# kije/gpu_raytracer

Hardware: AMD Instinct MI355X
Metric: Mrays/s (higher is better)
Workload: dtype f32

## Files before the change

### gpu_raytracer_amd/csrc/wavefront.hip

```cpp
#include "wavefront.h"
#include <cstdlib>

#include <algorithm>

#include "device_common.h"

using namespace rtdev;

#ifndef RT_WF_REFILL
#define RT_WF_REFILL 16
#endif
#ifndef RT_WF_CHUNK
#define RT_WF_CHUNK 256
#endif
#ifndef RT_WF_ADAPTIVE_CHUNK
#define RT_WF_ADAPTIVE_CHUNK 1
#endif
#ifndef RT_WF_WINDOW
#define RT_WF_WINDOW 512
#endif
#ifndef RT_WF_BLOCK_MAJOR
#define RT_WF_BLOCK_MAJOR 1
#endif
#ifndef RT_WF_SHADE_WAVES
// ... 346 lines not shown
        unsigned long long n0 = wave_sum(cnt.nodes), n1 = wave_sum(cnt.tris);
        for (int off = 32; off > 0; off >>= 1) sp_max = max(sp_max, __shfl_down(sp_max, off, WAVE));
        if (lane == 0) {
            atomicAdd(&wb.totals[rt::WF_TOTAL_NODE_VISITS], n0);
            atomicAdd(&wb.totals[rt::WF_TOTAL_TRI_TESTS], n1);
            atomicMax(&wb.totals[rt::WF_TOTAL_STACK_MAX], (unsigned long long)sp_max);
            atomicAdd(&wb.totals[rt::WF_TOTAL_NODE_STEPS], (unsigned long long)d_node_steps);
            atomicAdd(&wb.totals[rt::WF_TOTAL_LEAF_STEPS], (unsigned long long)d_leaf_steps);
            atomicAdd(&wb.totals[rt::WF_TOTAL_LEAF_LANES], (unsigned long long)d_leaf_lanes);
            atomicAdd(&wb.totals[rt::WF_TOTAL_LEAF_TRIPS], (unsigned long long)d_leaf_trips);
            atomicAdd(&wb.totals[rt::WF_TOTAL_REFILLS], (unsigned long long)d_refills);
        }
        const unsigned long long e0 = wave_sum(d_empty), e1 = wave_sum(d_entered);
        if (lane == 0) {
            atomicAdd(&wb.totals[rt::WF_TOTAL_EMPTY_VISITS], e0);
            atomicAdd(&wb.totals[rt::WF_TOTAL_CHILDREN_ENTERED], e1);
        }
    }
}

#ifndef RT_BEAM_STACK
#define RT_BEAM_STACK 512
#endif
#ifndef RT_BEAM_LEAVES
#define RT_BEAM_LEAVES 1024
#endif
#ifndef RT_BEAM_MARGIN_PX
#define RT_BEAM_MARGIN_PX 0.125f
#endif
#ifndef RT_BEAM_SAMPLES_PER_WAVE
#define RT_BEAM_SAMPLES_PER_WAVE 8u
#endif
#ifndef RT_BEAM_DIST_SCALE
#define RT_BEAM_DIST_SCALE 0.99999f
#endif
#ifndef RT_BEAM_EARLY_OUT
#define RT_BEAM_EARLY_OUT 1
#endif
#ifndef RT_BEAM_TRI_CULL
#define RT_BEAM_TRI_CULL 1
#endif
struct BeamPlanes {
    V3 n[4];
    V3 o;
};
__device__ __forceinline__ bool beam_outside(const BeamPlanes& bp, const float lo[3], const float hi[3]) {
    bool outside = false;
    for (int k = 0; k < 4; k++) {
        const V3 pv = v3((bp.n[k].x > 0.0f ? hi[0] : lo[0]) - bp.o.x, (bp.n[k].y > 0.0f ? hi[1] : lo[1]) - bp.o.y, (bp.n[k].z > 0.0f ? hi[2] : lo[2]) - bp.o.z);
        outside = outside || dot(bp.n[k], pv) < 0.0f;
    }
    return outside;
}
__device__ __forceinline__ float beam_box_distance(const V3 o, const float lo[3], const float hi[3]) {
    const float dx = fmaxf(fmaxf(lo[0] - o.x, o.x - hi[0]), 0.0f), dy = fmaxf(fmaxf(lo[1] - o.y, o.y - hi[1]), 0.0f), dz = fmaxf(fmaxf(lo[2] - o.z, o.z - hi[2]), 0.0f);
    return sqrtf(dx * dx + dy * dy + dz * dz) * RT_BEAM_DIST_SCALE;
}
__global__ __launch_bounds__(WAVE) void k_wf_beams(DevScene sc, DevFrame fr, rt::WfBuffers wb) {
    __shared__ uint32_t s_nodes[RT_BEAM_STACK];
    __shared__ uint32_t s_leaf[RT_BEAM_LEAVES];
    __shared__ uint32_t s_ref[RT_BEAM_CAP];
    __shared__ float s_dist[RT_BEAM_CAP];
    const uint32_t lane = threadIdx.x, b = blockIdx.x;
    const PixelCoord p0 = block_pixel_at(fr, b, 0);
    const float x0 = (float)p0.x - RT_BEAM_MARGIN_PX, x1 = (float)p0.x + 8.0f + RT_BEAM_MARGIN_PX;
    const float y0 = (float)p0.y - RT_BEAM_MARGIN_PX, y1 = (float)p0.y + 8.0f + RT_BEAM_MARGIN_PX;
    const DevCamera& cam = fr.cam;
    auto dir = [&](float sx, float sy) {
        const float u = sx / cam.width_f, v = sy / cam.height_f;
        const float cx = (u * 2.0f - 1.0f) * cam.aspect * cam.fov_scale, cy = (1.0f - v * 2.0f) * cam.fov_scale;
        return ld3(cam.forward) + ld3(cam.right) * cx + ld3(cam.true_up) * cy;
    };
    const V3 cs[4] = {dir(x0, y0), dir(x1, y0), dir(x1, y1), dir(x0, y1)};
    const V3 cc = dir(0.5f * (x0 + x1), 0.5f * (y0 + y1));
    BeamPlanes bp;
    bp.o = ld3(cam.origin);
    bool bad = false;
    for (int k = 0; k < 4; k++) {
        bp.n[k] = cross(cs[k], cs[(k + 1) & 3]);
        const float s = dot(bp.n[k], cc);
        if (s < 0.0f) bp.n[k] = -bp.n[k];
        for (int j = 0; j < 4; j++)
            bad = bad || !(dot(bp.n[k], cs[j]) >= -1e-6f * (fabsf(bp.n[k].x) + fabsf(bp.n[k].y) + fabsf(bp.n[k].z)) * (fabsf(cs[j].x) + fabsf(cs[j].y) + fabsf(cs[j].z)));
        bad = bad || !(fabsf(s) > 0.0f) || !(fabsf(s) < RT_F32_MAX);
    }
    uint32_t n_stack = 0, n_leaf = 0;
    bool overflow = bad;
    if (sc.n_nodes) {
        if (lane == 0) s_nodes[0] = 0u;
        n_stack = 1;
    }
    __syncthreads();
    const uint32_t slot = lane & 7u;
    const unsigned long long lower = (1ull << lane) - 1ull;
    while (n_stack > 0 && !overflow) {
        const uint32_t take = min(n_stack, 8u), base = n_stack - take;
        const bool have = (lane >> 3) < take;
        const uint32_t node = have ? s_nodes[base + (lane >> 3)] : 0u;
        __syncthreads();
        n_stack = base;
        bool inner = false, leaf = false;
        uint32_t ref = 0;
        if (have) {
            const DevNode8& nd = sc.nodes[node];
            const uint32_t ex = nd.ex_imask, imask = ex >> 24, lmask = nd.lmask & 0xFFu;
            if (((imask | lmask) >> slot) & 1u) {
                float lo[3], hi[3];
                for (int a = 0; a < 3; a++) {
                    const float sca = ldexpf(1.0f, (int)(int8_t)((ex >> (8 * a)) & 0xFFu));
                    const float ql = (float)((nd.qlo[a][slot >> 2] >> (8u * (slot & 3u))) & 0xFFu), qh = (float)((nd.qhi[a][slot >> 2] >> (8u * (slot & 3u))) & 0xFFu);
                    lo[a] = nd.org[a] + ql * sca;
                    hi[a] = nd.org[a] + qh * sca;
                    const float pad = (fabsf(lo[a]) + fabsf(hi[a])) * 2.0e-6f + 1.0e-30f;
                    lo[a] -= pad;
                    hi[a] += pad;
                }
                if (!beam_outside(bp, lo, hi)) {
                    const uint32_t below = (1u << slot) - 1u;
                    if ((imask >> slot) & 1u) {
                        inner = true;
                        ref = nd.child_base + (uint32_t)__popc(imask & below);
                    } else {
                        leaf = true;
                        ref = nd.tri_base + RT_DEV_LEAF_STRIDE * (uint32_t)__popc(lmask & below);
                    }
                }
            }
        }
        const unsigned long long mi = __ballot(inner), ml = __ballot(leaf);
        const uint32_t pi = n_stack + (uint32_t)__popcll(mi & lower), pc = n_leaf + (uint32_t)__popcll(ml & lower);
        if (inner && pi < RT_BEAM_STACK) s_nodes[pi] = ref;
        if (leaf && pc < RT_BEAM_LEAVES) s_leaf[pc] = ref;
        n_stack += (uint32_t)__popcll(mi);
        n_leaf += (uint32_t)__popcll(ml);
        overflow = n_stack > RT_BEAM_STACK || n_leaf > RT_BEAM_LEAVES;
        __syncthreads();
    }
    uint32_t n_tri = 0;
    for (uint32_t l0 = 0; l0 < n_leaf && !overflow; l0 += WAVE) {
        const uint32_t li = l0 + lane;
        uint32_t first = 0, count = 0;
        if (li < n_leaf) {
            first = s_leaf[li];
            count = sc.tris[first].leaf_count;
        }
        for (uint32_t k = 0; k < RT_DEV_LEAF_STRIDE; k++) {
            bool keep = false;
            float dist = 0.0f;
            if (k < count) {
                const DevTri& t = sc.tris[first + k];
                float lo[3], hi[3];
                for (int a = 0; a < 3; a++) {
                    const float va = t.v0[a], vb = t.v0[a] + t.e1[a], vc = t.v0[a] + t.e2[a];
                    lo[a] = fminf(va, fminf(vb, vc));
                    hi[a] = fmaxf(va, fmaxf(vb, vc));
                    const float pad = (fabsf(lo[a]) + fabsf(hi[a])) * 2.0e-6f + 1.0e-30f;
                    lo[a] -= pad;
                    hi[a] += pad;
                }
                keep = !RT_BEAM_TRI_CULL || !(lo[0] <= hi[0] && lo[1] <= hi[1] && lo[2] <= hi[2]) || !beam_outside(bp, lo, hi);
                dist = beam_box_distance(bp.o, lo, hi);
                if (!(dist >= 0.0f)) dist = 0.0f;
            }
            const unsigned long long mk = __ballot(keep);
            const uint32_t pos = n_tri + (uint32_t)__popcll(mk & lower);
            if (keep && pos < RT_BEAM_CAP) {
                s_ref[pos] = first + k;
                s_dist[pos] = dist;
            }
            n_tri += (uint32_t)__popcll(mk);
        }
        overflow = n_tri > RT_BEAM_CAP;
    }
    __syncthreads();
    if (overflow) {
        if (lane == 0) wb.beam_count[b] = RT_BEAM_OVERFLOW | atomicAdd(&wb.beam_count[wb.n_blocks], 1u);
        return;
    }
    for (uint32_t i = lane; i < n_tri; i += WAVE) {
        const float di = s_dist[i];
        uint32_t rank = 0;
        for (uint32_t j = 0; j < n_tri; j++) {
            const float dj = s_dist[j];
            rank += (dj < di || (dj == di && j < i)) ? 1u : 0u;
        }
        wb.beam_ref[(size_t)b * RT_BEAM_CAP + rank] = s_ref[i];
        wb.beam_dist[(size_t)b * RT_BEAM_CAP + rank] = di;
    }
    if (lane == 0) wb.beam_count[b] = n_tri;
}

template <bool COUNT>
__global__ __launch_bounds__(WAVE) void k_wf_trace_camera(DevScene sc, rt::WfBuffers wb, uint32_t n_samples) {
    extern __shared__ uint4 s_cam[];
    if (wb.totals[rt::WF_TOTAL_ERROR] != 0ull) return;
    const uint32_t lane = threadIdx.x;
    float* s_d = reinterpret_cast<float*>(s_cam + RT_BEAM_CAP * 3u);
    Counts cnt = {0u, 0u};
    const uint32_t chunks = (n_samples + RT_BEAM_SAMPLES_PER_WAVE - 1u) / RT_BEAM_SAMPLES_PER_WAVE;
    for (uint32_t item = blockIdx.x; item < wb.n_blocks * chunks; item += gridDim.x) {
        const uint32_t b = item / chunks, k_first = (item - b * chunks) * RT_BEAM_SAMPLES_PER_WAVE, k_end = min(n_samples, k_first + RT_BEAM_SAMPLES_PER_WAVE);
        const uint32_t n_list = (uint32_t)__builtin_amdgcn_readfirstlane((int)wb.beam_count[b]);
        if (n_list & RT_BEAM_OVERFLOW) continue;
        {
            __syncthreads();
            for (uint32_t i = lane; i < n_list; i += WAVE) {
                const uint32_t slot = wb.beam_ref[(size_t)b * RT_BEAM_CAP + i];
                const uint4* __restrict__ rec = reinterpret_cast<const uint4*>(sc.tris + slot);
                const uint4 q0 = rec[0], q1 = rec[1], q2 = rec[2];
                s_cam[3u * i] = q0;
                s_cam[3u * i + 1u] = q1;
                s_cam[3u * i + 2u] = make_uint4(q2.x, q2.y, q2.z, slot);
                s_d[i] = wb.beam_dist[(size_t)b * RT_BEAM_CAP + i];
            }
            __syncthreads();
        }
        for (uint32_t k = k_first; k < k_end; k++) {
            const uint32_t sb = RT_WF_BLOCK_MAJOR ? b * n_samples + k : k * wb.n_blocks + b;
            const uint32_t p = sb * WAVE + lane;
            const bool valid = wb.pxy[p] != 0xFFFFFFFFu;
            if (__ballot(valid) == 0ull) continue;
            V3 o = v3(0.0f, 0.0f, 0.0f), d = v3(0.0f, 0.0f, 1.0f);
            if (valid) {
                float4 ro = wb.ray_o[p], rd = wb.ray_d[p];
                RT_KEEP4_EARLY(ro);
                RT_KEEP4_EARLY(rd);
                o = f4v(ro);
                d = f4v(rd);
            }
            Hit hit;
            hit.t = valid ? RT_F32_MAX : -1.0f;
            hit.prim = RT_PRIM_MISS;
            hit.slot = 0;
            if (valid) test_spheres(sc, o, d, hit, RT_MIN_RAY_DISTANCE);
            {
                for (uint32_t i = 0; i < n_list; i++) {
                    if (RT_BEAM_EARLY_OUT && __ballot(s_d[i] < hit.t) == 0ull) break;
                    const uint4 q0 = s_cam[3u * i], q1 = s_cam[3u * i + 1u], q2 = s_cam[3u * i + 2u];
                    if (COUNT && valid) cnt.tris++;
                    float t = 0.0f;
                    const bool inside = moller_trumbore(v3(__uint_as_float(q0.x), __uint_as_float(q0.y), __uint_as_float(q0.z)), v3(__uint_as_float(q0.w), __uint_as_float(q1.x), __uint_as_float(q1.y)),
                                                        v3(__uint_as_float(q1.z), __uint_as_float(q1.w), __uint_as_float(q2.x)), o, d, t);
                    const uint32_t prim = q2.z;
                    const bool accept = inside && t > RT_MIN_RAY_DISTANCE && (t < hit.t || (t == hit.t && prim < hit.prim && hit.prim < RT_PRIM_SPHERE_FLAG));
                    hit.t = accept ? t : hit.t;
                    hit.prim = accept ? prim : hit.prim;
                    hit.slot = accept ? q2.w : hit.slot;
                }
            }
            if (COUNT && wb.probe == 2u && valid) {
                Hit h2;
                h2.t = RT_F32_MAX;
                h2.prim = RT_PRIM_MISS;
                h2.slot = 0;
                Counts c2 = {0u, 0u};
                test_spheres(sc, o, d, h2, RT_MIN_RAY_DISTANCE);
                traverse<false, false>(sc, o, d, reinterpret_cast<uint2*>(s_cam + RT_BEAM_CAP * 4u) + lane, h2, c2, RT_MIN_RAY_DISTANCE);
                if (h2.prim != hit.prim || h2.t != hit.t) {
                    if (atomicAdd(&wb.totals[rt::WF_TOTAL_EMPTY_VISITS], 1ull) == 0ull) {
                        wb.totals[rt::WF_TOTAL_NODE_STEPS] = b;
                        wb.totals[rt::WF_TOTAL_LEAF_STEPS] = ((unsigned long long)hit.prim << 32) | h2.prim;
                        wb.totals[rt::WF_TOTAL_LEAF_LANES] = ((unsigned long long)__float_as_uint(hit.t) << 32) | __float_as_uint(h2.t);
                        wb.totals[rt::WF_TOTAL_LEAF_TRIPS] = ((unsigned long long)n_list << 32) | h2.slot;
                        wb.totals[rt::WF_TOTAL_REFILLS] = p;
                    }
                }
            }
            if (valid) {
                const V3 hp = o + d * hit.t;
                const uint32_t code = hit.prim == RT_PRIM_MISS ? RT_PRIM_MISS : ((hit.prim & RT_PRIM_SPHERE_FLAG) ? hit.prim : hit.slot);
                wb.hit[p] = make_uint4(__float_as_uint(hp.x), __float_as_uint(hp.y), __float_as_uint(hp.z), code);
            }
        }
    }
    if (COUNT) {
        const unsigned long long n0 = wave_sum(cnt.nodes), n1 = wave_sum(cnt.tris);
        if (lane == 0) {
            atomicAdd(&wb.totals[rt::WF_TOTAL_NODE_VISITS], n0);
            atomicAdd(&wb.totals[rt::WF_TOTAL_TRI_TESTS], n1);
        }
    }
}

#define RT_KEEP4(v) asm volatile("" : "+v"((v).x), "+v"((v).y), "+v"((v).z), "+v"((v).w))
__device__ __forceinline__ void stage_lights(DevLight* __restrict__ s_lights, const DevScene& sc) {
    const uint32_t words = sc.n_lights * (uint32_t)(sizeof(DevLight) / 4);
    const uint32_t* __restrict__ src = reinterpret_cast<const uint32_t*>(sc.lights);
    uint32_t* dst = reinterpret_cast<uint32_t*>(s_lights);
    for (uint32_t i = threadIdx.x; i < words; i += blockDim.x) dst[i] = src[i];
    __syncthreads();
}
__device__ __forceinline__ DevMaterial load_material(const DevScene& sc, uint32_t material_id) {
    const float4* p = reinterpret_cast<const float4*>(sc.materials + material_id);
    float4 a = p[0], b = p[1];
    RT_KEEP4(a);
    RT_KEEP4(b);
    DevMaterial m;
    m.albedo[0] = a.x; m.albedo[1] = a.y; m.albedo[2] = a.z; m.metallic = a.w;
    m.emission[0] = b.x; m.emission[1] = b.y; m.emission[2] = b.z; m.ior = b.w;
    const float2 c = *reinterpret_cast<const float2*>(reinterpret_cast<const float*>(sc.materials + material_id) + 8);
    m.transmission = c.x; m.roughness = c.y;
    m._pad[0] = m._pad[1] = 0.0f;
    return m;
}

#ifndef RT_WF_GRID_WALK
#define RT_WF_GRID_WALK 31
#endif
static_assert(EXT_EPS == RT_SG_EXT_EPS, "the light grids' dilation is derived from the shadow segments' origin offset");
static_assert(RT_WF_GRID_WALK < RT_SG_SORTED_PREFIX, "a walk may only look at the ordered part of a list");
#ifndef RT_WF_GRID_BLOCKS_PER_CU
#define RT_WF_GRID_BLOCKS_PER_CU 32
#endif
#ifndef RT_WF_GRID_MIN_WAVES
#define RT_WF_GRID_MIN_WAVES 7
#endif
enum : uint32_t { GRID_VISIBLE = 0u, GRID_OCCLUDED = 1u, GRID_FORWARD = 2u, GRID_PENDING = 3u };
struct GridPending {
    V3 o, d;
    float dist, limit;
    uint32_t at;
    uint32_t i, count;
};
static_assert(RT_SG_BLOCK_ENTRIES == 2u, "grid_segment_head tests the block's two entries by name");
template <bool COUNT>
__device__ __forceinline__ uint32_t grid_segment_head(const DevScene& sc, const DevLight& light, const DevShadowGrid& g, V3 point, V3 normal, GridPending& pend,
                                                      uint32_t& n_tests, uint32_t& n_entries) {
    V3 d;
    float dist;
    shadow_segment(light, point, d, dist);
    const V3 o = point + normal * EXT_EPS;
    Hit hit;
    hit.t = dist;
    hit.prim = RT_PRIM_MISS;
    hit.slot = 0;
    test_spheres(sc, o, d, hit, RT_MIN_RAY_DISTANCE);
    if (hit.prim != RT_PRIM_MISS) return GRID_OCCLUDED;
    const uint32_t kind = g.kind;
    uint32_t cell = 0xFFFFFFFFu;
    float limit = 0.0f;
    if (kind == RT_SG_KIND_CUBE) {
        const float wx = -d.x, wy = -d.y, wz = -d.z;
        const float ax = fabsf(wx), ay = fabsf(wy), az = fabsf(wz);
        const uint32_t a = (ax >= ay && ax >= az) ? 0u : (ay >= az ? 1u : 2u);
        const float wa = a == 0u ? wx : (a == 1u ? wy : wz), wb_ = a == 0u ? wy : (a == 1u ? wz : wx), wc = a == 0u ? wz : (a == 1u ? wx : wy);
        const float inv = __builtin_amdgcn_rcpf(fabsf(wa));
        const float fu = (wb_ * inv + 1.0f) * g.scale, fv = (wc * inv + 1.0f) * g.scale;
        const uint32_t top = g.res - 1u;
        const uint32_t ix = min((uint32_t)max((int)floorf(fu), 0), top), iy = min((uint32_t)max((int)floorf(fv), 0), top);
        cell = ((2u * a + (wa < 0.0f ? 1u : 0u)) * g.res + iy) * g.res + ix;
        limit = dist + g.limit_margin;
    } else if (kind == RT_SG_KIND_ORTHO) {
        const float fu = (dot(o, ld3(g.axis_u)) - g.u0) * g.scale, fv = (dot(o, ld3(g.axis_v)) - g.v0) * g.scale;
        const float r = (float)g.res;
        if (fu >= 0.0f && fu < r && fv >= 0.0f && fv < r) cell = (uint32_t)fv * g.res + (uint32_t)fu;
        limit = (g.key_top - dot(o, ld3(g.axis_w))) + g.limit_margin;
    } else {
        return GRID_FORWARD;
    }
    if (cell == 0xFFFFFFFFu && g.near_begin == g.near_end) return GRID_VISIBLE;
    uint4 hd = make_uint4(0u, 0u, 0x7F800000u, 0u), q0 = hd, q1 = hd, q2 = hd;
    const uint4* __restrict__ blk = g.blocks + (size_t)(cell == 0xFFFFFFFFu ? 0u : cell) * RT_SG_BLOCK_QUADS;
    if (cell != 0xFFFFFFFFu) {
        hd = blk[0];
        q0 = blk[1], q1 = blk[2], q2 = blk[3];
        RT_KEEP4(hd);
        RT_KEEP4(q0);
        RT_KEEP4(q1);
        RT_KEEP4(q2);
    }
    const uint32_t count = hd.x;
    if (count > g.heavy) return GRID_FORWARD;
    const uint4* __restrict__ ovf = g.overflow;
    for (uint32_t k = g.near_begin; k < g.near_end; k++) {
        const uint4 n0 = ovf[3 * (size_t)k], n1 = ovf[3 * (size_t)k + 1], n2 = ovf[3 * (size_t)k + 2];
        if (COUNT) n_tests++;
        float t;
        if (moller_trumbore(v3(__uint_as_float(n0.y), __uint_as_float(n0.z), __uint_as_float(n0.w)), v3(__uint_as_float(n1.x), __uint_as_float(n1.y), __uint_as_float(n1.z)),
                            v3(__uint_as_float(n1.w), __uint_as_float(n2.x), __uint_as_float(n2.y)), o, d, t) &&
            t > RT_MIN_RAY_DISTANCE && t < dist)
            return GRID_OCCLUDED;
    }
    if (count == 0u || !(__uint_as_float(q0.x) < limit)) return GRID_VISIBLE;
    float t;
    if (COUNT) n_entries++, n_tests++;
    if (moller_trumbore(v3(__uint_as_float(q0.y), __uint_as_float(q0.z), __uint_as_float(q0.w)), v3(__uint_as_float(q1.x), __uint_as_float(q1.y), __uint_as_float(q1.z)),
                        v3(__uint_as_float(q1.w), __uint_as_float(q2.x), __uint_as_float(q2.y)), o, d, t) &&
        t > RT_MIN_RAY_DISTANCE && t < dist)
        return GRID_OCCLUDED;
    if (count == 1u) return GRID_VISIBLE;
    q0 = blk[4], q1 = blk[5], q2 = blk[6];
    if (!(__uint_as_float(q0.x) < limit)) return GRID_VISIBLE;
    if (COUNT) n_entries++, n_tests++;
    if (moller_trumbore(v3(__uint_as_float(q0.y), __uint_as_float(q0.z), __uint_as_float(q0.w)), v3(__uint_as_float(q1.x), __uint_as_float(q1.y), __uint_as_float(q1.z)),
                        v3(__uint_as_float(q1.w), __uint_as_float(q2.x), __uint_as_float(q2.y)), o, d, t) &&
        t > RT_MIN_RAY_DISTANCE && t < dist)
        return GRID_OCCLUDED;
    if (count == 2u || !(__uint_as_float(hd.z) < limit)) return GRID_VISIBLE;
    pend.o = o, pend.d = d, pend.dist = dist, pend.limit = limit;
    pend.at = hd.y, pend.i = 2u, pend.count = count;
    return GRID_PENDING;
}
template <bool COUNT>
__device__ __forceinline__ uint32_t grid_walk_on(const DevShadowGrid& g, GridPending& pend, uint32_t trips, uint32_t& n_tests, uint32_t& n_entries) {
    const uint4* __restrict__ ovf = g.overflow;
    for (uint32_t k = 0; k < trips; k++) {
        const size_t at = 3 * (size_t)pend.at;
        uint4 q0 = ovf[at], q1 = ovf[at + 1], q2 = ovf[at + 2];
        RT_KEEP4(q0);
        RT_KEEP4(q1);
        RT_KEEP4(q2);
        if (!(__uint_as_float(q0.x) < pend.limit)) return GRID_VISIBLE;
        if (COUNT) n_entries++, n_tests++;
        float t;
        if (moller_trumbore(v3(__uint_as_float(q0.y), __uint_as_float(q0.z), __uint_as_float(q0.w)), v3(__uint_as_float(q1.x), __uint_as_float(q1.y), __uint_as_float(q1.z)),
                            v3(__uint_as_float(q1.w), __uint_as_float(q2.x), __uint_as_float(q2.y)), pend.o, pend.d, t) &&
            t > RT_MIN_RAY_DISTANCE && t < pend.dist)
            return GRID_OCCLUDED;
        pend.at++;
        pend.i++;
        if (pend.i >= pend.count) return GRID_VISIBLE;
        if (pend.i >= RT_WF_GRID_WALK) return GRID_FORWARD;
    }
    return GRID_PENDING;
}

#ifndef RT_WF_GRID_PASS
#define RT_WF_GRID_PASS 3u
#endif
#define RT_WF_GRID_PARK 128u
#define RT_WF_GRID_PARK_WORDS 11u
template <bool COUNT>
__global__ __launch_bounds__(256, RT_WF_GRID_MIN_WAVES) void k_wf_shadow_grid(DevScene sc, rt::WfBuffers wb, const uint32_t* __restrict__ queue) {
    __shared__ DevLight s_lights[RT_WF_MAX_LIGHTS];
    __shared__ DevShadowGrid s_grids[RT_WF_MAX_LIGHTS];
    __shared__ uint32_t s_fwd[4][128];
    __shared__ uint32_t s_park[4][RT_WF_GRID_PARK_WORDS][RT_WF_GRID_PARK];
    if (wb.totals[rt::WF_TOTAL_ERROR] != 0ull) return;
    const uint32_t lane = threadIdx.x & 63u, wave = threadIdx.x >> 6;
    const unsigned long long below = (1ull << lane) - 1ull;
    uint32_t n_fwd = 0, n_park = 0;
    stage_lights(s_lights, sc);
    {
        const uint32_t words = sc.n_lights * (uint32_t)(sizeof(DevShadowGrid) / 4);
        const uint32_t* __restrict__ src = reinterpret_cast<const uint32_t*>(wb.grids);
        uint32_t* dst = reinterpret_cast<uint32_t*>(s_grids);
        for (uint32_t i = threadIdx.x; i < words; i += blockDim.x) dst[i] = src[i];
        __syncthreads();
    }
    uint32_t n_tests = 0, n_entries = 0, n_answered = 0;
    uint32_t(*park)[RT_WF_GRID_PARK] = s_park[wave];
    auto hand_on = [&](bool forward, uint32_t entry, bool flush) {
        const unsigned long long fm = __ballot(forward);
        if (fm != 0ull) {
            if (forward) s_fwd[wave][n_fwd + (uint32_t)__popcll(fm & below)] = entry;
            n_fwd += (uint32_t)__popcll(fm);
        }
        if (n_fwd >= 64u || (flush && n_fwd)) {
            uint32_t at = 0;
            if (lane == 0) at = atomicAdd(&wb.counters[rt::WF_SHADOW2_COUNT], n_fwd);
            at = __shfl(at, 0, WAVE);
            for (uint32_t k = lane; k < n_fwd; k += WAVE) wb.q_shadow2[at + k] = s_fwd[wave][k];
            n_fwd = 0;
        }
    };
    auto park_push = [&](bool pending, const GridPending& pd, uint32_t entry) {
        const unsigned long long pm = __ballot(pending);
        if (pm == 0ull) return;
        if (pending) {
            const uint32_t s = n_park + (uint32_t)__popcll(pm & below);
            park[0][s] = __float_as_uint(pd.o.x), park[1][s] = __float_as_uint(pd.o.y), park[2][s] = __float_as_uint(pd.o.z);
            park[3][s] = __float_as_uint(pd.d.x), park[4][s] = __float_as_uint(pd.d.y), park[5][s] = __float_as_uint(pd.d.z);
            park[6][s] = __float_as_uint(pd.dist), park[7][s] = __float_as_uint(pd.limit);
            park[8][s] = pd.at, park[9][s] = pd.i | (pd.count << 8), park[10][s] = entry;
        }
        n_park += (uint32_t)__popcll(pm);
    };
    auto walk_parked = [&]() {
        const uint32_t take = min(n_park, 64u), first = n_park - take;
        const bool have = lane < take;
        GridPending pd = {};
        uint32_t entry = 0, outcome = GRID_VISIBLE;
        if (have) {
            const uint32_t s = first + lane;
            pd.o = v3(__uint_as_float(park[0][s]), __uint_as_float(park[1][s]), __uint_as_float(park[2][s]));
            pd.d = v3(__uint_as_float(park[3][s]), __uint_as_float(park[4][s]), __uint_as_float(park[5][s]));
            pd.dist = __uint_as_float(park[6][s]), pd.limit = __uint_as_float(park[7][s]);
            pd.at = park[8][s];
            const uint32_t ic = park[9][s];
            pd.i = ic & 0xFFu, pd.count = ic >> 8;
            entry = park[10][s];
            outcome = grid_walk_on<COUNT>(s_grids[entry >> 27], pd, RT_WF_GRID_PASS, n_tests, n_entries);
            if (outcome == GRID_OCCLUDED) atomicAnd(reinterpret_cast<uint32_t*>(&wb.vtx[2 * (size_t)(entry & RT_WF_ID_MASK) + 1]) + 3, ~(1u << (entry >> 27)));
            if (COUNT && outcome <= GRID_OCCLUDED) n_answered++;
        }
        n_park = first;
        park_push(have && outcome == GRID_PENDING, pd, entry);
        hand_on(have && outcome == GRID_FORWARD, entry, false);
    };
    const uint32_t count = wb.counters[rt::WF_EXT_COUNT];
    const uint32_t stride = gridDim.x * blockDim.x;
    uint32_t id_next = blockIdx.x * blockDim.x + threadIdx.x < count ? queue[blockIdx.x * blockDim.x + threadIdx.x] : WF_SENTINEL;
    for (uint32_t base = blockIdx.x * blockDim.x; base < count; base += stride) {
        const uint32_t id = id_next;
        const uint32_t i_next = base + stride + threadIdx.x;
        id_next = i_next < count ? queue[i_next] : WF_SENTINEL;
        uint32_t want = 0;
        V3 point = v3(0, 0, 0), normal = point;
        if (id != WF_SENTINEL) {
            float4 vp = wb.vtx[2 * (size_t)id], vn = wb.vtx[2 * (size_t)id + 1];
            RT_KEEP4(vp);
            RT_KEEP4(vn);
            point = f4v(vp), normal = f4v(vn);
            if (__float_as_uint(vp.w) != 0xFFFFFFFFu) want = __float_as_uint(vn.w);
        }
        uint32_t occluded = 0;
        for (uint32_t li = 0; li < sc.n_lights; li++) {
            const bool mine = (want >> li) & 1u;
            if (__ballot(mine) == 0ull) continue;
            uint32_t outcome = GRID_VISIBLE;
            GridPending pd = {};
            if (mine) {
                outcome = grid_segment_head<COUNT>(sc, s_lights[li], s_grids[li], point, normal, pd, n_tests, n_entries);
                if (outcome == GRID_OCCLUDED) occluded |= 1u << li;
                if (COUNT && outcome <= GRID_OCCLUDED) n_answered++;
            }
            const uint32_t entry = id | (li << 27);
            park_push(mine && outcome == GRID_PENDING, pd, entry);
            hand_on(mine && outcome == GRID_FORWARD, entry, false);
            while (n_park >= 64u) walk_parked();
        }
        if (occluded != 0u) atomicAnd(reinterpret_cast<uint32_t*>(&wb.vtx[2 * (size_t)id + 1]) + 3, ~occluded);
    }
    while (n_park != 0u) walk_parked();
    hand_on(false, 0u, true);
    if (COUNT) {
        const unsigned long long t = wave_sum(n_tests), a = wave_sum(n_answered), en = wave_sum(n_entries);
        if ((threadIdx.x & 63u) == 0) {
            atomicAdd(&wb.totals[rt::WF_TOTAL_TRI_TESTS], t);
            atomicAdd(&wb.totals[rt::WF_TOTAL_GRID_ANSWERED], a);
            atomicAdd(&wb.totals[rt::WF_TOTAL_GRID_ENTRIES], en);
        }
    }
}

__device__ __forceinline__ void wf_end_path(const rt::WfBuffers& wb, uint32_t id, V3 radiance) {
    wb.sample_rad[id] = make_float4(radiance.x, radiance.y, radiance.z, 0.0f);
}

__global__ __launch_bounds__(256, RT_WF_SHADE_WAVES) void k_wf_shade(DevScene sc, DevFrame fr, rt::WfBuffers wb, const uint32_t* __restrict__ queue) {
    __shared__ DevLight s_lights[RT_WF_MAX_LIGHTS];
    if (wb.totals[rt::WF_TOTAL_ERROR] != 0ull) return;
    stage_lights(s_lights, sc);
    const uint32_t count = wb.counters[rt::WF_EXT_COUNT];
    const bool shadows = (fr.flags & RT_FLAG_NO_SHADOWS) == 0;
    const bool to_grids = shadows && wb.grids != nullptr;
    const uint32_t stride = gridDim.x * blockDim.x;
    OutWindow win = {0u, 0u};
    uint32_t n_shadow = 0;
    const uint32_t window = pick_window((count + stride - 1u) / stride, max(1u, sc.n_lights));
    if (blockIdx.x == 0 && threadIdx.x == 0) wb.counters[rt::WF_SHADOW_WINDOW] = window;
    uint32_t id_next = blockIdx.x * blockDim.x + threadIdx.x < count ? queue[blockIdx.x * blockDim.x + threadIdx.x] : WF_SENTINEL;
    for (uint32_t base = blockIdx.x * blockDim.x; base < count; base += stride) {
        const uint32_t id = id_next;
        const uint32_t i_next = base + stride + threadIdx.x;
        id_next = i_next < count ? queue[i_next] : WF_SENTINEL;
        const bool have = id != WF_SENTINEL;
        bool vertex = false;
        V3 point = v3(0, 0, 0), normal = point;
        uint32_t material_id = 0;
        DevMaterial m = {};
        if (have) {
            uint4 h = wb.hit[id];
            asm volatile("" : "+v"(h.x), "+v"(h.y), "+v"(h.z), "+v"(h.w));
            if (h.w == RT_PRIM_MISS) {
                const V3 radiance = f4v(wb.rad[id]) + v3(0.1f, 0.2f, 0.3f) * f4v(wb.thr[id]);
                wf_end_path(wb, id, radiance);
            } else {
                point = v3(__uint_as_float(h.x), __uint_as_float(h.y), __uint_as_float(h.z));
                surface_at(sc, (h.w & RT_PRIM_SPHERE_FLAG) != 0, h.w & ~RT_PRIM_SPHERE_FLAG, point, normal, material_id);
                if (material_id >= sc.n_materials) {
                    const V3 radiance = f4v(wb.rad[id]) + v3(1.0f, 0.0f, 1.0f) * f4v(wb.thr[id]);
                    wf_end_path(wb, id, radiance);
                } else {
                    vertex = true;
                    m = load_material(sc, material_id);
                    wb.vtx[2 * (size_t)id] = make_float4(point.x, point.y, point.z, __uint_as_float(material_id));
                    if (!shadows) wb.vtx[2 * (size_t)id + 1] = make_float4(normal.x, normal.y, normal.z, 0.0f);
                }
            }
        }
        if (have && !vertex) wb.vtx[2 * (size_t)id] = make_float4(0.0f, 0.0f, 0.0f, __uint_as_float(0xFFFFFFFFu));
        if (shadows) {
            uint32_t mask = 0;
            if (vertex) {
                for (uint32_t li = 0; li < sc.n_lights; li++) {
                    V3 sdir;
                    float sdist;
                    const V3 contrib = light_contribution(s_lights[li], m, point, normal, sdir, sdist);
                    if (contrib.x != 0.0f || contrib.y != 0.0f || contrib.z != 0.0f) mask |= 1u << li;
                }
            }
            if (vertex) wb.vtx[2 * (size_t)id + 1] = make_float4(normal.x, normal.y, normal.z, __uint_as_float(mask));
            if (to_grids) {
                n_shadow += (uint32_t)__popc(mask);
                continue;
            }
#if RT_WF_SHADOW_LIGHT_MAJOR
            uint32_t total = 0;
            for (uint32_t li = 0; li < sc.n_lights; li++) total += (uint32_t)__popcll(__ballot((mask >> li) & 1u));
            if (total) {
                uint32_t at = window_reserve(wb.q_shadow, &wb.counters[rt::WF_SHADOW_COUNT], win, window, 0u, 0u, total, wb.q_shadow_cap, &wb.totals[rt::WF_TOTAL_ERROR]);
                n_shadow += (uint32_t)__popc(mask);
                const unsigned long long below = (1ull << (threadIdx.x & 63u)) - 1ull;
                for (uint32_t li = 0; at != WF_NO_SLOT && li < sc.n_lights; li++) {
                    const bool want = (mask >> li) & 1u;
                    const unsigned long long b = __ballot(want);
                    if (want) wb.q_shadow[at + (uint32_t)__popcll(b & below)] = id | (li << 27);
                    at += (uint32_t)__popcll(b);
                }
            }
#else
            const uint32_t mine = (uint32_t)__popc(mask);
            const uint32_t incl = wave_incl_scan(mine), total = __shfl(incl, WAVE - 1, WAVE);
            if (total) {
                uint32_t at = window_reserve(wb.q_shadow, &wb.counters[rt::WF_SHADOW_COUNT], win, window, mine, incl, total, wb.q_shadow_cap, &wb.totals[rt::WF_TOTAL_ERROR]);
                n_shadow += mine;
                while (mask && at != WF_NO_SLOT) {
                    const uint32_t li = (uint32_t)__ffs((int)mask) - 1u;
                    mask &= mask - 1u;
                    wb.q_shadow[at++] = id | (li << 27);
                }
            }
#endif
        }
    }
    window_close(wb.q_shadow, win);
    const unsigned long long ns = wave_sum(n_shadow);
    if ((threadIdx.x & 63u) == 0 && ns) atomicAdd(&wb.totals[rt::WF_TOTAL_SHADOW], ns);
}

__global__ void k_wf_advance(rt::WfBuffers wb) {
    if (threadIdx.x != 0 || blockIdx.x != 0) return;
    uint32_t* c = wb.counters;
    c[rt::WF_EXT_COUNT] = c[rt::WF_EXT_NEXT];
    c[rt::WF_EXT_WINDOW] = c[rt::WF_EXT_WINDOW_NEXT];
    c[rt::WF_EXT_NEXT] = 0;
    c[rt::WF_SHADOW_COUNT] = 0;
    c[rt::WF_SHADOW2_COUNT] = 0;
    c[rt::WF_SHADOW2_CURSOR] = 0;
    c[rt::WF_EXT_CURSOR] = 0;
    c[rt::WF_SHADOW_CURSOR] = 0;
}

__global__ __launch_bounds__(256, RT_WF_SHADE_WAVES) void k_wf_finish(DevScene sc, DevFrame fr, rt::WfBuffers wb, const uint32_t* __restrict__ queue,
                                                  uint32_t* __restrict__ next_queue) {
    __shared__ DevLight s_lights[RT_WF_MAX_LIGHTS];
    if (wb.totals[rt::WF_TOTAL_ERROR] != 0ull) return;
    stage_lights(s_lights, sc);
    const uint32_t count = wb.counters[rt::WF_EXT_COUNT];
    const bool shadows = (fr.flags & RT_FLAG_NO_SHADOWS) == 0;
    const uint32_t stride = gridDim.x * blockDim.x;
    OutWindow win = {0u, 0u};
    uint32_t n_cont = 0;
    const uint32_t window = pick_window((count + stride - 1u) / stride, 1u);
    if (blockIdx.x == 0 && threadIdx.x == 0) wb.counters[rt::WF_EXT_WINDOW_NEXT] = window;
    uint32_t id_next = blockIdx.x * blockDim.x + threadIdx.x < count ? queue[blockIdx.x * blockDim.x + threadIdx.x] : WF_SENTINEL;
    for (uint32_t base = blockIdx.x * blockDim.x; base < count; base += stride) {
        bool cont = false;
        const uint32_t id = id_next;
        const uint32_t i_next = base + stride + threadIdx.x;
        id_next = i_next < count ? queue[i_next] : WF_SENTINEL;
        float4 vp = make_float4(0.0f, 0.0f, 0.0f, __uint_as_float(0xFFFFFFFFu));
        float4 vn = vp, th = vp, ra = vp, rdin = vp;
        if (id != WF_SENTINEL) {
            vp = wb.vtx[2 * (size_t)id];
            vn = wb.vtx[2 * (size_t)id + 1];
            th = wb.thr[id];
            ra = wb.rad[id];
            rdin = wb.ray_d[id];
            RT_KEEP4(vp);
            RT_KEEP4(vn);
            RT_KEEP4(th);
            RT_KEEP4(ra);
            RT_KEEP4(rdin);
        }
        const uint32_t vis = __float_as_uint(vn.w);
        if (__float_as_uint(vp.w) != 0xFFFFFFFFu) {
            const V3 point = f4v(vp), normal = f4v(vn);
            const uint32_t material_id = __float_as_uint(vp.w);
            const DevMaterial m = load_material(sc, material_id);
            V3 throughput = f4v(th), radiance = f4v(ra);
            const uint32_t tw = __float_as_uint(th.w);
            uint32_t channel = tw & 0xFFu;
            const uint32_t depth = tw >> 8;
            SimpleRng rng = {__float_as_uint(ra.w)};
            const bool terminal = depth >= fr.max_bounce;
            V3 lighting = v3(0.0f, 0.0f, 0.0f);
            if (terminal) lighting = lighting + ld3(m.albedo) * 0.1f;
            for (uint32_t li = 0; li < sc.n_lights; li++) {
                V3 sdir;
                float sdist;
                const V3 contrib = light_contribution(s_lights[li], m, point, normal, sdir, sdist);
                const bool nonzero = contrib.x != 0.0f || contrib.y != 0.0f || contrib.z != 0.0f;
                if (nonzero && shadows && !((vis >> li) & 1u)) continue;
                lighting = lighting + contrib;
            }
            lighting = lighting + ld3(m.emission);
            const float tf = fminf(fmaxf(m.transmission, 0.0f), 1.0f);
            if (terminal) {
                V3 out = lighting;
                if (tf > 0.0f) out = transmission_mix(m, lighting, tf);
                radiance = radiance + out * throughput;
                wf_end_path(wb, id, radiance);
            } else {
                radiance = radiance + (lighting * (1.0f - tf)) * throughput;
                const V3 din = f4v(rdin);
                const bool front = dot(normal, din) < 0.0f;
                const V3 nf = front ? normal : -normal;
                bool transmit = false;
                if (tf > 0.0f) transmit = rng.next_f32() < tf;
                V3 ndir, norigin;
                const V3 albedo = ld3(m.albedo);
                bool absorbed = false;
                if (transmit) {
                    if (channel == 3) {
                        uint32_t c = (uint32_t)(rng.next_f32() * 3.0f);
                        channel = c < 2 ? c : 2;
                        throughput = v3(channel == 0 ? throughput.x * 3.0f : 0.0f, channel == 1 ? throughput.y * 3.0f : 0.0f,
                                        channel == 2 ? throughput.z * 3.0f : 0.0f);
                    }
                    const float offs = channel == 0 ? -0.018f : (channel == 1 ? 0.0f : 0.035f);
                    const float ior_c = m.ior + offs;
                    const float eta = front ? (1.0f / ior_c) : ior_c;
                    const float cos_i = -dot(nf, din);
                    const float sin2_t = eta * eta * (1.0f - cos_i * cos_i);
                    if (sin2_t > 1.0f) {
                        ndir = din - nf * (2.0f * dot(din, nf));
                        norigin = point + nf * EXT_EPS;
                    } else {
                        const float cos_t = sqrtf(1.0f - sin2_t);
                        ndir = din * eta + nf * (eta * cos_i - cos_t);
                        norigin = point - nf * EXT_EPS;
                    }
                    ndir = normalize(ndir);
                    throughput = throughput * albedo;
                } else if (m.metallic > 0.5f) {
                    const float u1 = rng.next_f32(), u2 = rng.next_f32();
                    const V3 r = din - nf * (2.0f * dot(din, nf));
                    ndir = normalize(r + unit_vector(u1, u2) * m.roughness);
                    absorbed = !(dot(ndir, nf) > 0.0f);
                    norigin = point + nf * EXT_EPS;
                    if (!absorbed) throughput = throughput * albedo;
                } else {
                    const float u1 = rng.next_f32(), u2 = rng.next_f32();
                    V3 w = nf + unit_vector(u1, u2);
                    if (dot(w, w) < 1e-12f) w = nf;
                    ndir = normalize(w);
                    norigin = point + nf * EXT_EPS;
                    throughput = throughput * albedo;
                }
                if (!absorbed && depth >= 2) {
                    const float p = fminf(fmaxf(fmaxf(fmaxf(throughput.x, throughput.y), throughput.z), 0.05f), 1.0f);
                    if (rng.next_f32() > p) absorbed = true;
                    else throughput = v3(throughput.x / p, throughput.y / p, throughput.z / p);
                }
                if (absorbed) {
                    wf_end_path(wb, id, radiance);
                } else {
                    cont = true;
                    wb.ray_o[id] = make_float4(norigin.x, norigin.y, norigin.z, 0.0f);
                    wb.ray_d[id] = make_float4(ndir.x, ndir.y, ndir.z, 0.0f);
                    wb.thr[id] = make_float4(throughput.x, throughput.y, throughput.z, __uint_as_float(channel | ((depth + 1u) << 8)));
                    wb.rad[id] = make_float4(radiance.x, radiance.y, radiance.z, __uint_as_float(rng.seed));
                }
            }
        }
        const uint32_t mine = cont ? 1u : 0u;
        const uint32_t incl = wave_incl_scan(mine), total = __shfl(incl, WAVE - 1, WAVE);
        if (total) {
            const uint32_t at = window_reserve(next_queue, &wb.counters[rt::WF_EXT_NEXT], win, window, mine, incl, total, wb.q_ext_cap, &wb.totals[rt::WF_TOTAL_ERROR]);
            if (cont && at != WF_NO_SLOT) next_queue[at] = id;
            n_cont += mine;
        }
    }
    window_close(next_queue, win);
    const unsigned long long nc = wave_sum(n_cont);
    if ((threadIdx.x & 63u) == 0 && nc) atomicAdd(&wb.totals[rt::WF_TOTAL_CONTINUATION], nc);
}

__global__ __launch_bounds__(WAVE) void k_wf_resolve(DevFrame fr, rt::WfBuffers wb, DevTargets tg, uint32_t n_samples, uint32_t first_batch,
                                                     uint32_t last_batch) {
    const uint32_t lane = threadIdx.x, b = blockIdx.x;
    const uint32_t q = b * WAVE + lane;
    float4 acc = first_batch ? make_float4(0.0f, 0.0f, 0.0f, 0.0f) : wb.accum[q];
    V3 sum = f4v(acc);
    for (uint32_t k = 0; k < n_samples; k++) sum = sum + f4v(wb.sample_rad[(size_t)(RT_WF_BLOCK_MAJOR ? b * n_samples + k : k * wb.n_blocks + b) * WAVE + lane]);
    wb.accum[q] = make_float4(sum.x, sum.y, sum.z, 0.0f);
    if (!last_batch) return;
    const PixelCoord px = block_pixel_at(fr, b, lane);
    if (!px.valid) return;
    const float n = (float)fr.spp;
    const V3 color = v3(sum.x / n, sum.y / n, sum.z / n);
    const size_t pix = (size_t)px.y * fr.width + px.x;
    if (tg.rgba32f) reinterpret_cast<float4*>(tg.rgba32f)[pix] = make_float4(color.x, color.y, color.z, 1.0f);
    if (tg.chan[0]) reinterpret_cast<uint32_t*>(tg.chan[0])[pix] = unorm8(color.x) | 0xFF000000u;
    if (tg.chan[1]) reinterpret_cast<uint32_t*>(tg.chan[1])[pix] = (unorm8(color.y) << 8) | 0xFF000000u;
    if (tg.chan[2]) reinterpret_cast<uint32_t*>(tg.chan[2])[pix] = (unorm8(color.z) << 16) | 0xFF000000u;
}

int g_cu_count = 0;
int cu_count() {
    if (g_cu_count == 0) {
        int dev = 0;
        hipDeviceProp_t prop;
        if (hipGetDevice(&dev) == hipSuccess && hipGetDeviceProperties(&prop, dev) == hipSuccess) g_cu_count = prop.multiProcessorCount;
        if (g_cu_count <= 0) g_cu_count = 256;
    }
    return g_cu_count;
}

}

namespace rt {

#ifndef RT_WF_SHADE_BLOCKS_PER_CU
#define RT_WF_SHADE_BLOCKS_PER_CU 16
#endif
uint32_t wf_shading_blocks() {
    static const int per_cu = [] {
        const char* e = std::getenv("RT_WF_SHADE_BLOCKS_PER_CU");
        const int v = e ? std::atoi(e) : 0;
        return v > 0 && v <= 64 ? v : RT_WF_SHADE_BLOCKS_PER_CU;
    }();
    return (uint32_t)(cu_count() * per_cu);
}
size_t wf_queue_slots_for(size_t max_entries, uint32_t per_lane, size_t waves) {
    return max_entries * 4 + (waves + 1) * 2 * ((size_t)wf_min_window(per_lane) + 64u * per_lane) + RT_WF_WINDOW_MAX;
}
size_t wf_queue_slots(size_t max_entries, uint32_t per_lane) { return wf_queue_slots_for(max_entries, per_lane, (size_t)wf_shading_blocks() * 4); }
uint32_t wf_pick_window(uint32_t iters, uint32_t per_lane) { return pick_window(iters, per_lane); }
uint32_t wf_persistent_waves() { return (uint32_t)(cu_count() * RT_WF_WAVES_PER_CU); }
static uint32_t trace_waves_per_cu(uint32_t path_slots) {
    static const int forced = [] { const char* e = std::getenv("RT_WF_WAVES_PER_CU"); const int v = e ? std::atoi(e) : 0; return v > 0 && v <= RT_WF_WAVES_PER_CU ? v : 0; }();
    if (forced) return (uint32_t)forced;
    return path_slots >= (24u << 20) ? (uint32_t)RT_WF_WAVES_PER_CU : RT_WF_WAVES_SMALL;
}

hipError_t wf_beams(const DevScene& sc, const DevFrame& fr, const WfBuffers& wb, hipStream_t s) {
    if (!wb.beam_count || wb.n_blocks == 0) return hipSuccess;
    const hipError_t e = hipMemsetAsync(wb.beam_count + wb.n_blocks, 0, sizeof(uint32_t), s);
    if (e != hipSuccess) return e;
    hipLaunchKernelGGL(k_wf_beams, dim3(wb.n_blocks), dim3(WAVE), 0, s, sc, fr, wb);
    return hipGetLastError();
}

hipError_t wf_generate(const DevScene&, const DevFrame& fr, const WfBuffers& wb, uint32_t first_sample, uint32_t n_samples, hipStream_t s) {
    hipError_t e = hipMemsetAsync(wb.counters, 0, WF_N_COUNTERS * sizeof(uint32_t), s);
    if (e != hipSuccess) return e;
    if (wb.n_blocks == 0 || n_samples == 0) return hipSuccess;
    hipLaunchKernelGGL(k_wf_generate, dim3(wf_shading_blocks()), dim3(256), 0, s, fr, wb, first_sample, n_samples * wb.n_blocks);
    return hipGetLastError();
}

template <bool COUNT, bool ANY>
static void launch_trace(const DevScene& sc, const WfBuffers& wb, const uint32_t* q, uint32_t count_slot, uint32_t cursor_slot, uint32_t window_slot, hipStream_t s) {
    const size_t lds = (size_t)RT_WF8_LDS_STACK * WAVE * sizeof(uint2) + 2048;
    hipLaunchKernelGGL((k_wf_trace<COUNT, ANY>), dim3((uint32_t)cu_count() * trace_waves_per_cu(wb.capacity)), dim3(WAVE), lds, s, sc, wb, q, count_slot, cursor_slot, window_slot);
}

hipError_t wf_bounce(const DevScene& sc, const DevFrame& fr, const WfBuffers& wb, uint32_t iteration, uint32_t n_samples, bool counters, hipStream_t s, hipEvent_t* grid_events) {
    const dim3 sgrid(wf_shading_blocks()), sblock(256);
    uint32_t* cur_q = wb.q_ext[iteration & 1u];
    uint32_t* next_q = wb.q_ext[(iteration + 1u) & 1u];
    if (iteration == 0 && wb.beam_count && n_samples && wb.n_blocks) {
        const dim3 lgrid(std::min<uint32_t>(wb.n_blocks * ((n_samples + RT_BEAM_SAMPLES_PER_WAVE - 1u) / RT_BEAM_SAMPLES_PER_WAVE), (uint32_t)cu_count() * 96u));
        const size_t list_lds = (size_t)RT_BEAM_CAP * (3 * sizeof(uint4) + sizeof(float)), walk_lds = (size_t)std::max(1u, sc.stack_entries) * WAVE * sizeof(uint2);
        if (counters) {
            hipLaunchKernelGGL((k_wf_trace_camera<true>), lgrid, dim3(WAVE), wb.probe == 2u ? (size_t)RT_BEAM_CAP * 64 + walk_lds : list_lds, s, sc, wb, n_samples);
            launch_trace<true, false>(sc, wb, wb.q_ext[1], WF_FB_COUNT, WF_FB_CURSOR, WF_SHADOW2_WINDOW, s);
        } else {
            hipLaunchKernelGGL((k_wf_trace_camera<false>), lgrid, dim3(WAVE), list_lds, s, sc, wb, n_samples);
            launch_trace<false, false>(sc, wb, wb.q_ext[1], WF_FB_COUNT, WF_FB_CURSOR, WF_SHADOW2_WINDOW, s);
        }
    } else if (counters) launch_trace<true, false>(sc, wb, cur_q, WF_EXT_COUNT, WF_EXT_CURSOR, WF_EXT_WINDOW, s);
    else launch_trace<false, false>(sc, wb, cur_q, WF_EXT_COUNT, WF_EXT_CURSOR, WF_EXT_WINDOW, s);
    hipLaunchKernelGGL(k_wf_shade, sgrid, sblock, 0, s, sc, fr, wb, (const uint32_t*)cur_q);
    if (wf_runs_shadow_grid(fr, wb)) {
        const dim3 ggrid((uint32_t)(cu_count() * RT_WF_GRID_BLOCKS_PER_CU));
        if (grid_events) (void)hipEventRecord(grid_events[0], s);
        if (counters) hipLaunchKernelGGL(k_wf_shadow_grid<true>, ggrid, dim3(256), 0, s, sc, wb, (const uint32_t*)cur_q);
        else hipLaunchKernelGGL(k_wf_shadow_grid<false>, ggrid, dim3(256), 0, s, sc, wb, (const uint32_t*)cur_q);
        if (grid_events) (void)hipEventRecord(grid_events[1], s);
        if (counters) launch_trace<true, true>(sc, wb, wb.q_shadow2, WF_SHADOW2_COUNT, WF_SHADOW2_CURSOR, WF_SHADOW2_WINDOW, s);
        else launch_trace<false, true>(sc, wb, wb.q_shadow2, WF_SHADOW2_COUNT, WF_SHADOW2_CURSOR, WF_SHADOW2_WINDOW, s);
    } else if ((fr.flags & RT_FLAG_NO_SHADOWS) == 0) {
        if (counters) launch_trace<true, true>(sc, wb, wb.q_shadow, WF_SHADOW_COUNT, WF_SHADOW_CURSOR, WF_SHADOW_WINDOW, s);
        else launch_trace<false, true>(sc, wb, wb.q_shadow, WF_SHADOW_COUNT, WF_SHADOW_CURSOR, WF_SHADOW_WINDOW, s);
    }
    hipLaunchKernelGGL(k_wf_finish, sgrid, sblock, 0, s, sc, fr, wb, (const uint32_t*)cur_q, next_q);
    hipLaunchKernelGGL(k_wf_advance, dim3(1), dim3(1), 0, s, wb);
    return hipGetLastError();
}

hipError_t wf_resolve(const DevFrame& fr, const WfBuffers& wb, const DevTargets& tg, uint32_t n_samples, bool first_batch, bool last_batch, hipStream_t s) {
    if (wb.n_blocks == 0) return hipSuccess;
    hipLaunchKernelGGL(k_wf_resolve, dim3(wb.n_blocks), dim3(WAVE), 0, s, fr, wb, tg, n_samples, first_batch ? 1u : 0u, last_batch ? 1u : 0u);
    return hipGetLastError();
}

}
```

Before: 2914.

## Fuse shading into the shadow-grid kernel when light grids are active

When the shadow-grid path runs, the separate shade launch is dropped. The grid kernel now reads the hit record itself, computes the surface and material, finds which lights contribute, writes the vertex buffers and ends missed paths. This removes one kernel launch and the round trip of vertex data through global memory between shade and grid. In exchange the grid kernel carries more register and compute load, which may lower occupancy, and it adds an explicit vmcnt wait before the light loop.

```diff
diff --git a/gpu_raytracer_amd/csrc/wavefront.hip b/gpu_raytracer_amd/csrc/wavefront.hip
--- a/gpu_raytracer_amd/csrc/wavefront.hip
+++ b/gpu_raytracer_amd/csrc/wavefront.hip
@@ -672,6 +672,9 @@
     m.transmission = c.x; m.roughness = c.y;
     m._pad[0] = m._pad[1] = 0.0f;
     return m;
+}
+__device__ __forceinline__ void wf_end_path(const rt::WfBuffers& wb, uint32_t id, V3 radiance) {
+    wb.sample_rad[id] = make_float4(radiance.x, radiance.y, radiance.z, 0.0f);
 }
 
 #ifndef RT_WF_GRID_WALK
@@ -800,6 +803,7 @@
 #endif
 #define RT_WF_GRID_PARK 128u
 #define RT_WF_GRID_PARK_WORDS 11u
+#define RT_WAITCNT_VMCNT0 0x0F70
 template <bool COUNT>
 __global__ __launch_bounds__(256, RT_WF_GRID_MIN_WAVES) void k_wf_shadow_grid(DevScene sc, rt::WfBuffers wb, const uint32_t* __restrict__ queue) {
     __shared__ DevLight s_lights[RT_WF_MAX_LIGHTS];
@@ -818,7 +822,7 @@
         for (uint32_t i = threadIdx.x; i < words; i += blockDim.x) dst[i] = src[i];
         __syncthreads();
     }
-    uint32_t n_tests = 0, n_entries = 0, n_answered = 0;
+    uint32_t n_tests = 0, n_entries = 0, n_answered = 0, n_shadow = 0;
     uint32_t(*park)[RT_WF_GRID_PARK] = s_park[wave];
     auto hand_on = [&](bool forward, uint32_t entry, bool flush) {
         const unsigned long long fm = __ballot(forward);
@@ -830,6 +834,7 @@
             uint32_t at = 0;
             if (lane == 0) at = atomicAdd(&wb.counters[rt::WF_SHADOW2_COUNT], n_fwd);
             at = __shfl(at, 0, WAVE);
+#pragma unroll 1
             for (uint32_t k = lane; k < n_fwd; k += WAVE) wb.q_shadow2[at + k] = s_fwd[wave][k];
             n_fwd = 0;
         }
@@ -878,12 +883,37 @@
         uint32_t want = 0;
         V3 point = v3(0, 0, 0), normal = point;
         if (id != WF_SENTINEL) {
-            float4 vp = wb.vtx[2 * (size_t)id], vn = wb.vtx[2 * (size_t)id + 1];
-            RT_KEEP4(vp);
-            RT_KEEP4(vn);
-            point = f4v(vp), normal = f4v(vn);
-            if (__float_as_uint(vp.w) != 0xFFFFFFFFu) want = __float_as_uint(vn.w);
-        }
+            bool vertex = false;
+            uint4 h = wb.hit[id];
+            asm volatile("" : "+v"(h.x), "+v"(h.y), "+v"(h.z), "+v"(h.w));
+            if (h.w == RT_PRIM_MISS) {
+                const V3 radiance = f4v(wb.rad[id]) + v3(0.1f, 0.2f, 0.3f) * f4v(wb.thr[id]);
+                wf_end_path(wb, id, radiance);
+            } else {
+                point = v3(__uint_as_float(h.x), __uint_as_float(h.y), __uint_as_float(h.z));
+                uint32_t material_id = 0;
+                surface_at(sc, (h.w & RT_PRIM_SPHERE_FLAG) != 0, h.w & ~RT_PRIM_SPHERE_FLAG, point, normal, material_id);
+                if (material_id >= sc.n_materials) {
+                    const V3 radiance = f4v(wb.rad[id]) + v3(1.0f, 0.0f, 1.0f) * f4v(wb.thr[id]);
+                    wf_end_path(wb, id, radiance);
+                } else {
+                    vertex = true;
+                    const DevMaterial m = load_material(sc, material_id);
+                    wb.vtx[2 * (size_t)id] = make_float4(point.x, point.y, point.z, __uint_as_float(material_id));
+#pragma clang loop vectorize(disable) interleave(disable)
+                    for (uint32_t li = 0; li < sc.n_lights; li++) {
+                        V3 sdir;
+                        float sdist;
+                        const V3 contrib = light_contribution(s_lights[li], m, point, normal, sdir, sdist);
+                        if (contrib.x != 0.0f || contrib.y != 0.0f || contrib.z != 0.0f) want |= 1u << li;
+                    }
+                    wb.vtx[2 * (size_t)id + 1] = make_float4(normal.x, normal.y, normal.z, __uint_as_float(want));
+                }
+            }
+            if (!vertex) wb.vtx[2 * (size_t)id] = make_float4(0.0f, 0.0f, 0.0f, __uint_as_float(0xFFFFFFFFu));
+        }
+        n_shadow += (uint32_t)__popc(want);
+        __builtin_amdgcn_s_waitcnt(RT_WAITCNT_VMCNT0);
         uint32_t occluded = 0;
         for (uint32_t li = 0; li < sc.n_lights; li++) {
             const bool mine = (want >> li) & 1u;
@@ -904,6 +934,8 @@
     }
     while (n_park != 0u) walk_parked();
     hand_on(false, 0u, true);
+    const unsigned long long ns = wave_sum(n_shadow);
+    if ((threadIdx.x & 63u) == 0 && ns) atomicAdd(&wb.totals[rt::WF_TOTAL_SHADOW], ns);
     if (COUNT) {
         const unsigned long long t = wave_sum(n_tests), a = wave_sum(n_answered), en = wave_sum(n_entries);
         if ((threadIdx.x & 63u) == 0) {
@@ -914,9 +946,6 @@
     }
 }
 
-__device__ __forceinline__ void wf_end_path(const rt::WfBuffers& wb, uint32_t id, V3 radiance) {
-    wb.sample_rad[id] = make_float4(radiance.x, radiance.y, radiance.z, 0.0f);
-}
 
 __global__ __launch_bounds__(256, RT_WF_SHADE_WAVES) void k_wf_shade(DevScene sc, DevFrame fr, rt::WfBuffers wb, const uint32_t* __restrict__ queue) {
     __shared__ DevLight s_lights[RT_WF_MAX_LIGHTS];
@@ -924,7 +953,6 @@
     stage_lights(s_lights, sc);
     const uint32_t count = wb.counters[rt::WF_EXT_COUNT];
     const bool shadows = (fr.flags & RT_FLAG_NO_SHADOWS) == 0;
-    const bool to_grids = shadows && wb.grids != nullptr;
     const uint32_t stride = gridDim.x * blockDim.x;
     OutWindow win = {0u, 0u};
     uint32_t n_shadow = 0;
@@ -972,10 +1000,6 @@
                 }
             }
             if (vertex) wb.vtx[2 * (size_t)id + 1] = make_float4(normal.x, normal.y, normal.z, __uint_as_float(mask));
-            if (to_grids) {
-                n_shadow += (uint32_t)__popc(mask);
-                continue;
-            }
 #if RT_WF_SHADOW_LIGHT_MAJOR
             uint32_t total = 0;
             for (uint32_t li = 0; li < sc.n_lights; li++) total += (uint32_t)__popcll(__ballot((mask >> li) & 1u));
@@ -1255,7 +1279,6 @@
         }
     } else if (counters) launch_trace<true, false>(sc, wb, cur_q, WF_EXT_COUNT, WF_EXT_CURSOR, WF_EXT_WINDOW, s);
     else launch_trace<false, false>(sc, wb, cur_q, WF_EXT_COUNT, WF_EXT_CURSOR, WF_EXT_WINDOW, s);
-    hipLaunchKernelGGL(k_wf_shade, sgrid, sblock, 0, s, sc, fr, wb, (const uint32_t*)cur_q);
     if (wf_runs_shadow_grid(fr, wb)) {
         const dim3 ggrid((uint32_t)(cu_count() * RT_WF_GRID_BLOCKS_PER_CU));
         if (grid_events) (void)hipEventRecord(grid_events[0], s);
@@ -1264,9 +1287,12 @@
         if (grid_events) (void)hipEventRecord(grid_events[1], s);
         if (counters) launch_trace<true, true>(sc, wb, wb.q_shadow2, WF_SHADOW2_COUNT, WF_SHADOW2_CURSOR, WF_SHADOW2_WINDOW, s);
         else launch_trace<false, true>(sc, wb, wb.q_shadow2, WF_SHADOW2_COUNT, WF_SHADOW2_CURSOR, WF_SHADOW2_WINDOW, s);
-    } else if ((fr.flags & RT_FLAG_NO_SHADOWS) == 0) {
-        if (counters) launch_trace<true, true>(sc, wb, wb.q_shadow, WF_SHADOW_COUNT, WF_SHADOW_CURSOR, WF_SHADOW_WINDOW, s);
-        else launch_trace<false, true>(sc, wb, wb.q_shadow, WF_SHADOW_COUNT, WF_SHADOW_CURSOR, WF_SHADOW_WINDOW, s);
+    } else {
+        hipLaunchKernelGGL(k_wf_shade, sgrid, sblock, 0, s, sc, fr, wb, (const uint32_t*)cur_q);
+        if ((fr.flags & RT_FLAG_NO_SHADOWS) == 0) {
+            if (counters) launch_trace<true, true>(sc, wb, wb.q_shadow, WF_SHADOW_COUNT, WF_SHADOW_CURSOR, WF_SHADOW_WINDOW, s);
+            else launch_trace<false, true>(sc, wb, wb.q_shadow, WF_SHADOW_COUNT, WF_SHADOW_CURSOR, WF_SHADOW_WINDOW, s);
+        }
     }
     hipLaunchKernelGGL(k_wf_finish, sgrid, sblock, 0, s, sc, fr, wb, (const uint32_t*)cur_q, next_q);
     hipLaunchKernelGGL(k_wf_advance, dim3(1), dim3(1), 0, s, wb);
```

Result: faster. 2948, median of 6 (+1.2%).
